# humansensinglab/AGenDA

Hardware: AMD Instinct MI355X
Metric: 512x512 images/sec + DAAM heatmaps, 50 DDIM steps, SD-1.5 (higher is better)
Workload: dtype bf16

## Files before the change

### agenda_amd/_lib.py

```python
from __future__ import annotations

import ctypes as C
import os

_HERE = os.path.dirname(os.path.abspath(__file__))
LIB_PATH = os.environ.get("AGD_LIB") or os.path.join(_HERE, "libagenda_hip.so")
AGD_MAX_LEVELS = 8
AGD_N_CLASSES = 11


class AgdConfig(C.Structure):
    _fields_ = [
        ("struct_size", C.c_int),
        ("in_channels", C.c_int), ("out_channels", C.c_int), ("n_levels", C.c_int),
        ("block_out_channels", C.c_int * AGD_MAX_LEVELS),
        ("down_cross", C.c_int * AGD_MAX_LEVELS),
        ("num_heads", C.c_int * AGD_MAX_LEVELS),
        ("layers_per_block", C.c_int), ("cross_attention_dim", C.c_int),
        ("use_linear_projection", C.c_int), ("norm_num_groups", C.c_int),
        ("vae_latent_channels", C.c_int), ("vae_out_channels", C.c_int), ("vae_n_levels", C.c_int),
        ("vae_block_out_channels", C.c_int * AGD_MAX_LEVELS),
        ("vae_layers_per_block", C.c_int), ("vae_norm_num_groups", C.c_int),
        ("vae_scaling_factor", C.c_float),
        ("max_tokens", C.c_int),
# ... 158 lines not shown
    "agd_hook_num_maps": (C.c_int, [_P]),
    "agd_hook_map_dims": (C.c_int, [_P, C.c_int, C.POINTER(C.c_int)]),
    "agd_hook_map": (C.c_int, [_P, C.c_int, _P, _P]),
    "agd_op_attn_reg_loss": (C.c_int, [_P, C.c_int, C.c_int, C.c_int, _P, _P, _P, C.c_float, _P, _P, _P]),
    "agd_attn_processor_backward": (C.c_int, [_P, C.c_char_p, _P, _P, _P, _P, C.c_int, C.c_int, C.c_int, C.c_int, _P, _P, _P]),
    "agd_op_conv2d": (C.c_int, [_P, _P, _P, _P] + [C.c_int] * 9 + [_P]),
    "agd_op_conv2d_ex": (C.c_int, [_P, _P, _P, _P] + [C.c_int] * 10 + [_P]),
    "agd_op_linear": (C.c_int, [_P, _P, _P, _P, _P, C.c_int, C.c_int, C.c_int, C.c_int, _P]),
    "agd_op_groupnorm": (C.c_int, [_P, _P, _P, _P, C.c_int, C.c_int, C.c_int, C.c_int, C.c_float, C.c_int, _P]),
    "agd_op_groupnorm_ex": (C.c_int, [_P] * 5 + [C.c_int] * 5 + [C.c_float, C.c_int, _P, C.c_int, _P, C.c_int, C.POINTER(C.c_int), _P]),
    "agd_op_gn_fold": (C.c_int, [_P, _P] + [C.c_int] * 5 + [C.c_float] + [_P] * 4 + [C.c_int, C.c_int] + [_P] * 5 + [_P]),
    "agd_op_conv_groupnorm": (C.c_int, [_P] * 6 + [C.c_int] * 6 + [C.c_float, C.c_int, C.c_int, _P]),
    "agd_op_igemm": (C.c_int, [C.POINTER(AgdIgemmDesc), _P]),
    "agd_op_layernorm": (C.c_int, [_P, _P, _P, _P, C.c_int, C.c_int, C.c_float, _P]),
    "agd_op_layernorm_ex": (C.c_int, [_P, _P, _P, _P, C.c_int, C.c_int, C.c_float, C.POINTER(C.c_int), _P]),
    "agd_op_ff_fused": (C.c_int, [_P] * 8 + [C.c_int, C.c_int, C.c_float, _P]),
    "agd_op_attn_chain": (C.c_int, [_P] * 9 + [C.c_int] * 5 + [C.c_float, _P]),
    "agd_op_ff_fused_ex": (C.c_int, [_P] * 8 + [C.c_int, C.c_int, C.c_float, _P, _P, _P, C.c_int, _P, C.c_int, _P, C.c_int, _P]),
    "agd_op_attn_chain_ex": (C.c_int, [_P] * 8 + [C.c_int] * 5 + [C.c_float] + [_P] * 4 + [C.c_int, _P, _P] + [C.c_int] * 6 + [_P]),
    "agd_op_qkv_chain": (C.c_int, [_P] * 3 + [C.c_int, C.c_float, _P, C.c_int] + [_P] * 4 + [C.c_float] + [_P] * 3 + [C.c_int] * 4 + [_P]),
    "agd_op_xattn_premul": (C.c_int, [_P] * 9 + [C.c_int] * 5 + [C.c_float, _P]),
    "agd_op_attention": (C.c_int, [_P, _P, _P, _P, C.c_int, C.c_int, C.c_int, C.c_int, C.c_int, C.c_float, _P, _P]),
    "agd_op_attention_ex": (C.c_int, [_P, _P, _P, _P] + [C.c_int] * 5 + [C.c_float, C.c_int, _P, _P, _P, C.c_int, C.c_int, _P, C.c_int, C.c_int, C.c_int, _P]),
    "agd_op_attention_long": (C.c_int, [_P, _P, _P, _P] + [C.c_int] * 5 + [C.c_float, C.c_int, _P, C.c_int, C.c_int, _P]),
    "agd_op_attention_headsum": (C.c_int, [_P, _P, _P, _P, C.c_int, C.c_int, C.c_int, C.c_int, C.c_int, C.c_float, _P, _P]),
    "agd_op_attention_backward": (C.c_int, [_P, _P, _P, _P] + [C.c_int] * 6 + [C.c_float, _P, _P, _P]),
    "agd_op_hook_headmean": (C.c_int, [_P, C.c_int, C.c_int, C.c_int, C.c_int, _P, _P]),
    "agd_op_bicubic_clamp_mean": (C.c_int, [_P, C.c_int, C.c_int, C.c_int, C.c_int, _P, _P]),
    "agd_op_heatmap_u8": (C.c_int, [_P, C.c_int, C.c_int, _P, _P]),
    "agd_op_resize_u8_pil": (C.c_int, [_P, C.c_int, C.c_int, C.c_int, C.c_int, C.c_int, C.c_int, _P, _P]),
    "agd_op_stack_heatmaps": (C.c_int, [_P, _P, _P, C.c_longlong, _P, _P, _P]),
    "agd_op_window_gather": (C.c_int, [_P, _P] + [C.c_int] * 8 + [_P]),
    "agd_op_window_mean": (C.c_int, [_P, _P] + [C.c_int] * 6 + [_P]),
    "agd_denoise_panorama": (C.c_int, [_P, _P] + [C.c_int] * 7 + [C.POINTER(C.c_float)] * 3 + [C.c_float, _P]),
    "agd_daam_global_panorama": (C.c_int, [_P, C.c_int, C.c_int, _P, _P]),
    "agd_op_region_masks": (C.c_int, [_P, C.c_int, C.c_int, _P] + [C.c_int] * 6 + [_P]),
    "agd_op_region_spread": (C.c_int, [_P] * 5 + [C.c_int] * 6 + [C.POINTER(C.c_int), C.c_float, C.c_float, _P]),
    "agd_op_region_mean": (C.c_int, [_P, _P, _P] + [C.c_int] * 5 + [_P]),
    "agd_denoise_regions": (C.c_int, [_P, _P, C.c_int, C.c_int, C.c_int, C.POINTER(AgdRegionsDesc), C.c_int] + [C.POINTER(C.c_float)] * 3 + [C.c_float, _P]),
    "agd_freeu_set": (C.c_int, [_P] + [C.c_float] * 4),
    "agd_freeu_clear": (C.c_int, [_P]),
    "agd_freeu_counts": (C.c_int, [_P, C.POINTER(C.c_longlong)]),
    "agd_op_freeu": (C.c_int, [_P, _P, _P, _P] + [C.c_int] * 5 + [C.c_float, C.c_float, _P]),
    "agd_guidance_rescale_set": (C.c_int, [_P, C.c_float]),
    "agd_guidance_rescale_clear": (C.c_int, [_P]),
    "agd_guidance_rescale_counts": (C.c_int, [_P, C.POINTER(C.c_longlong)]),
# ... 56 lines not shown
```

### agenda_amd/csrc/attention.hip

```cpp
#include "kernels.h"
#include <type_traits>

#ifdef AGD_EXPERIMENTS
int g_attn_qb = 1;
extern "C" __attribute__((visibility("default"))) void agd_set_attn_qb(int v) { g_attn_qb = v; }
#else
constexpr int g_attn_qb = 1;
#endif

template <int D> struct AttnCfg {
  static constexpr int KSTEPS = (D + 15) / 16;
  static constexpr int DBLK = (D + 31) / 32;
  static constexpr int KCH = KSTEPS * 2;
  static constexpr int KPITCH = ((KCH | 1)) * 16;
  static constexpr int VPITCH = ((DBLK | 1)) * 64;
  static constexpr int CH = D / 8;
  static constexpr bool ONES = (DBLK * 32 > D);
  static constexpr bool QPAD = (KSTEPS * 16 > D);
};

#define DEFER_THR 8.0f

template <int D, int KB, int QB, int RECORD, int AMASK = 0, int EXTRA = 0>
#if defined(AGD_EXPERIMENTS) && defined(EXP_ATTN_LB)
#define ATTN_LB(def) ((!RECORD && !AMASK) ? EXP_ATTN_LB : (def))
#else
#define ATTN_LB(def) (def)
#endif
__global__ __launch_bounds__(256, ATTN_LB((AMASK ? 1 : (QB == 1 && D <= 64 && !RECORD) ? 3 : (QB == 1 && D <= 80) ? 2 : 1))) void attn_kernel(const AttnP p) {
  using C = AttnCfg<D>;
  constexpr int KEYS = KB * 32;
  constexpr int KSTEPS = C::KSTEPS, DBLK = C::DBLK, KPITCH = C::KPITCH, VPITCH = C::VPITCH, CH = C::CH;
  constexpr bool ONES = C::ONES && !RECORD;
  constexpr bool QPAD = C::QPAD && !RECORD;
  constexpr bool CNEG = !QPAD && !RECORD;
  constexpr int NCHUNK = KEYS * CH;
  constexpr int LD_IT = (NCHUNK + 255) / 256;
  constexpr int STAGE = KEYS * (KPITCH + VPITCH);
  constexpr int NSTAGE = (RECORD == 1) ? 1 : 2;
  extern __shared__ __attribute__((aligned(16))) char smem[];

  const int tid = threadIdx.x, lane = tid & 63, wid = tid >> 6;
  const int c = lane & 31, hh = lane >> 5;
  const int HPB = (RECORD == 2) ? p.H / p.rec_hpb : p.H;
  const int nqt = p.nqt, nbh = p.B * HPB;
  int bh, qt;
  {
    const int id = blockIdx.x, x = id & 7, j = id >> 3;
    const int per = (nbh + 7) >> 3;
    const int lb = j / nqt;
    qt = j - lb * nqt;
    bh = x * per + lb;
  }
  if (bh >= nbh) return;
  const int hgrp = bh % HPB;
  int head = (RECORD == 2) ? hgrp * p.rec_hpb : hgrp;
  const int hend = (RECORD == 2) ? head + p.rec_hpb : head + 1;
  const int b = bh / HPB;
  const int q0 = qt * (128 * QB) + wid * (32 * QB);
  const bf16_t* kp = p.k + b * p.sk + head * D;
  const bf16_t* vp = p.v + b * p.sv + head * D;

// ... 41 lines not shown
    const bf16_t* qp = p.q + b * p.sq + h * D;
    const int qrow = q0 + c;
#pragma unroll
    for (int s = 0; s < (RECORD == 2 ? KSTEPS : 1); ++s) {
      const int d0 = 16 * s + 8 * hh;
      qnext[s] = u32x4{0, 0, 0, 0};
      if (qrow < p.Nq && d0 < D) qnext[s] = *(const u32x4*)(qp + (long long)qrow * p.ldq + d0);
    }
  };
  load_q();

  u32x4 kreg[LD_IT], vreg[LD_IT];
  unsigned kvoff[LD_IT], vvoff[LD_IT];
#pragma unroll
  for (int it = 0; it < LD_IT; ++it) {
    const int idx = tid + it * 256;
    const int r = idx / CH, cc = idx - r * CH;
    kvoff[it] = (idx < NCHUNK) ? (unsigned)((r * p.ldk + cc * 8) * 2) : 0x80000000u;
    vvoff[it] = (idx < NCHUNK) ? (unsigned)((r * p.ldv + cc * 8) * 2) : 0x80000000u;
  }
  const unsigned k_bytes = (unsigned)(((long long)(p.Nk - 1) * p.ldk + D) * 2), v_bytes = (unsigned)(((long long)(p.Nk - 1) * p.ldv + D) * 2);
  const auto krs = __builtin_amdgcn_make_buffer_rsrc((void*)kp, 0, k_bytes, 0x00020000);
  const auto vrs = __builtin_amdgcn_make_buffer_rsrc((void*)vp, 0, v_bytes, 0x00020000);
  auto gload = [&](int tile) {
    const unsigned ks_ = __builtin_amdgcn_readfirstlane((unsigned)(tile * KEYS * p.ldk * 2));
    const unsigned vs_ = __builtin_amdgcn_readfirstlane((unsigned)(tile * KEYS * p.ldv * 2));
#pragma unroll
    for (int it = 0; it < LD_IT; ++it) {
      kreg[it] = __builtin_bit_cast(u32x4, __builtin_amdgcn_raw_buffer_load_b128(krs, kvoff[it], ks_, 0));
      vreg[it] = __builtin_bit_cast(u32x4, __builtin_amdgcn_raw_buffer_load_b128(vrs, vvoff[it], vs_, 0));
    }
  };
  auto gload_head = [&](int h) {
    const auto krh = __builtin_amdgcn_make_buffer_rsrc((void*)(p.k + b * p.sk + h * D), 0, k_bytes, 0x00020000);
    const auto vrh = __builtin_amdgcn_make_buffer_rsrc((void*)(p.v + b * p.sv + h * D), 0, v_bytes, 0x00020000);
#pragma unroll
    for (int it = 0; it < LD_IT; ++it) {
      kreg[it] = __builtin_bit_cast(u32x4, __builtin_amdgcn_raw_buffer_load_b128(krh, kvoff[it], 0, 0));
      vreg[it] = __builtin_bit_cast(u32x4, __builtin_amdgcn_raw_buffer_load_b128(vrh, vvoff[it], 0, 0));
    }
  };
  auto gload_extra = [&]() {
    const unsigned k2b = (unsigned)(((long long)(p.Nk2 - 1) * p.ldk2 + D) * 2), v2b = (unsigned)(((long long)(p.Nk2 - 1) * p.ldv2 + D) * 2);
    const auto kr2 = __builtin_amdgcn_make_buffer_rsrc((void*)(p.k2 + b * p.sk2 + head * D), 0, k2b, 0x00020000);
    const auto vr2 = __builtin_amdgcn_make_buffer_rsrc((void*)(p.v2 + b * p.sv2 + head * D), 0, v2b, 0x00020000);
#pragma unroll
// ... 30 lines not shown
  float m_run[QB], l_run[QB];
  [[maybe_unused]] bool seen[QB];
  f32x16 negm[CNEG ? QB : 1];
#pragma unroll
  for (int qb = 0; qb < QB; ++qb) {
    m_run[qb] = RECORD ? -INFINITY : 0.f; l_run[qb] = 0.f; seen[qb] = false;
    if constexpr (CNEG) {
#pragma unroll
      for (int j = 0; j < 16; ++j) negm[qb][j] = 0.f;
    }
  }
  const float sc = qscale;
  f32x16 pacc[RECORD == 2 ? KB : 1];
  const bool recb = RECORD == 2 && p.record_mode == 3 && b >= p.rec_b0;
  if constexpr (RECORD == 2) {
#pragma unroll
    for (int kb = 0; kb < KB; ++kb)
#pragma unroll
      for (int j = 0; j < 16; ++j) pacc[kb][j] = 0.f;
  }

  const int ntiles_main = RECORD ? 1 : (p.Nk + KEYS - 1) / KEYS;
  const int ntiles = ntiles_main + (EXTRA ? 1 : 0);
  const bool ragged = (p.Nk % KEYS) != 0 || p.causal || AMASK;
  gload(0);
  lstore(0);
  __syncthreads();

  const int gi = lane & 15;
  const int tr_row = (gi >> 2) + 4 * hh;
  const int tr_col = ((lane >> 4) & 1) * 16 + (gi & 3) * 4;

  auto tile_body = [&](int t, auto mask_tag) {
    constexpr bool MASK = decltype(mask_tag)::value;
    const int cur = (RECORD == 1) ? 0 : (RECORD == 2) ? ((t - (hend - p.rec_hpb)) & 1) : (t & 1);
    const char* sK = smem + cur * STAGE;
    const char* sV = sK + KEYS * KPITCH;
    if constexpr (RECORD == 2) { if (t + 1 < hend) { gload_head(t + 1); prefetch_q(t + 1); } }
    else if constexpr (EXTRA) { if (t + 1 < ntiles_main) gload(t + 1); else if (t + 1 == ntiles_main) gload_extra(); }
    else if (t + 1 < ntiles) gload(t + 1);
    f32x16 sacc[QB][KB];
#pragma unroll
    for (int kb = 0; kb < KB; ++kb) {
#pragma unroll
      for (int s = 0; s < KSTEPS; ++s) {
        const bf16x8 a = *(const bf16x8*)(sK + (kb * 32 + c) * KPITCH + (2 * s + hh) * 16);
#pragma unroll
        for (int qb = 0; qb < QB; ++qb) {
          if (s == 0) { const f32x16 z = {0.f, 0.f, 0.f, 0.f, 0.f, 0.f, 0.f, 0.f, 0.f, 0.f, 0.f, 0.f, 0.f, 0.f, 0.f, 0.f};
                        sacc[qb][kb] = __builtin_amdgcn_mfma_f32_32x32x16_bf16(a, qf[qb][s], CNEG ? negm[qb] : z, 0, 0, 0); }
          else sacc[qb][kb] = __builtin_amdgcn_mfma_f32_32x32x16_bf16(a, qf[qb][s], sacc[qb][kb], 0, 0, 0);
        }
      }
    }
    if constexpr (MASK) {
#pragma unroll
      for (int qb = 0; qb < QB; ++qb)
#pragma unroll
        for (int kb = 0; kb < KB; ++kb)
#pragma unroll
          for (int i = 0; i < 16; ++i) {
            const int key = (RECORD || (EXTRA && t == ntiles_main) ? 0 : t * KEYS) + kb * 32 + (i & 3) + 8 * (i >> 2) + 4 * hh;
// ... 95 lines not shown
          float* base = p.rec + img * p.rec_img_stride + head * p.rec_head_stride;
          const unsigned nbytes = (unsigned)p.rec_T * (unsigned)p.Nq * 4u;
          const auto rsrc = __builtin_amdgcn_make_buffer_rsrc(base, 0, nbytes, 0x00020000);
          const unsigned rowb = (unsigned)p.Nq * 4u;
          const unsigned voff0 = (unsigned)(q0 + c) * 4u + (unsigned)(4 * hh) * rowb;
#pragma unroll
          for (int kb = 0; kb < KB; ++kb) {
            float old[16];
#pragma unroll
            for (int i = 0; i < 16; ++i) {
              const unsigned off = voff0 + (unsigned)(kb * 32 + (i & 3) + 8 * (i >> 2)) * rowb;
              old[i] = __builtin_bit_cast(float, __builtin_amdgcn_raw_buffer_load_b32(rsrc, off, 0, 0));
            }
#pragma unroll
            for (int i = 0; i < 16; ++i) {
              const unsigned off = voff0 + (unsigned)(kb * 32 + (i & 3) + 8 * (i >> 2)) * rowb;
              __builtin_amdgcn_raw_buffer_store_b32(__builtin_bit_cast(unsigned, old[i] + sacc[0][kb][i] * inv), rsrc, off, 0, 0);
            }
          }
        }
      }
    }

#pragma unroll
    for (int kb = 0; kb < KB; ++kb)
#pragma unroll
      for (int s = 0; s < 2; ++s) {
        bf16x8 pf[QB];
#pragma unroll
        for (int qb = 0; qb < QB; ++qb)
#pragma unroll
          for (int j = 0; j < 8; ++j) pf[qb][j] = (__bf16)sacc[qb][kb][8 * s + j];
        const char* vb = sV + (kb * 32 + 16 * s + tr_row) * VPITCH + tr_col * 2;
#pragma unroll
        for (int db = 0; db < DBLK; ++db) {
          const s16x4 lo = __builtin_amdgcn_ds_read_tr16_b64_v4i16((__attribute__((address_space(3))) s16x4*)(vb + db * 64));
          const s16x4 hi = __builtin_amdgcn_ds_read_tr16_b64_v4i16((__attribute__((address_space(3))) s16x4*)(vb + 8 * VPITCH + db * 64));
          const u32x2 lo2 = __builtin_bit_cast(u32x2, lo), hi2 = __builtin_bit_cast(u32x2, hi);
          const u32x4 a4 = u32x4{lo2[0], lo2[1], hi2[0], hi2[1]};
#pragma unroll
          for (int qb = 0; qb < QB; ++qb)
            oacc[qb][db] = __builtin_amdgcn_mfma_f32_32x32x16_bf16(__builtin_bit_cast(bf16x8, a4), pf[qb], oacc[qb][db], 0, 0, 0);
        }
      }
    if ((RECORD == 2) ? (t + 1 < hend) : (t + 1 < ntiles)) {
      lstore(cur ^ 1);
      __syncthreads();
    }
  };
  auto store_o = [&]() {
#pragma unroll
    for (int qb = 0; qb < QB; ++qb) {
      float lt;
      if constexpr (ONES) {
        constexpr int ld = D % 32;
        const float lv = oacc[qb][D / 32][4 * (ld / 8)];
        lt = __shfl(lv, c);
      } else {
        lt = xhalf_sum(l_run[qb]);
      }
      const float inv = 1.0f / lt;
      const int qrow = q0 + qb * 32 + c;
      if (qrow < p.Nq) {
        bf16_t* op = p.o + b * p.so + (long long)qrow * p.ldo + head * D;
#pragma unroll
        for (int db = 0; db < DBLK; ++db)
#pragma unroll
          for (int g = 0; g < 4; ++g) {
            const int d0 = db * 32 + 8 * g + 4 * hh;
// ... 39 lines not shown
        for (int kb = 0; kb < KB; ++kb)
#pragma unroll
          for (int i = 0; i < 16; ++i)
            __builtin_amdgcn_raw_buffer_store_b32(__builtin_bit_cast(unsigned, old[kb][i] + pacc[kb][i]), rsrc,
                                                  voff0 + (unsigned)(kb * 32 + (i & 3) + 8 * (i >> 2)) * rowb, 0, 0);
      }
      return;
    } else if constexpr (RECORD) {
      tile_body(0, T_{});
    } else if constexpr (EXTRA) {
      for (int t = 0; t < ntiles_main - 1; ++t) tile_body(t, F_{});
      if (ragged) tile_body(ntiles_main - 1, T_{}); else tile_body(ntiles_main - 1, F_{});
      tile_body(ntiles_main, T_{});
    } else {
      if (p.causal || AMASK) { for (int t = 0; t < ntiles - 1; ++t) tile_body(t, T_{}); }
      else { for (int t = 0; t < ntiles - 1; ++t) tile_body(t, F_{}); }
      if (ragged) tile_body(ntiles - 1, T_{}); else tile_body(ntiles - 1, F_{});
    }
  }
  store_o();
}


template <int D, int KB, int QB, int RECORD, int AMASK = 0, int EXTRA = 0>
static int launch_attn_t(const AttnP& p, hipStream_t st) {
  using C = AttnCfg<D>;
  constexpr int lds = (RECORD == 1 ? 1 : 2) * KB * 32 * (C::KPITCH + C::VPITCH);
  AttnP pp = p;
  pp.nqt = (p.Nq + 128 * QB - 1) / (128 * QB);
  const int per = (p.B * (RECORD == 2 ? p.H / p.rec_hpb : p.H) + 7) / 8;
  dim3 grid(8 * per * pp.nqt);
  auto kfn = attn_kernel<D, KB, QB, RECORD, AMASK, EXTRA>;
  if (lds > 65536) {
    static std::atomic<bool> attr[AGD_MAX_DEVICES] = {};
    int dev = 0; HIP_CHECK_RET(hipGetDevice(&dev));
    if (dev < 0 || dev >= AGD_MAX_DEVICES) { agd_set_error("attention: device ordinal %d out of range", dev); return -1; }
    if (!attr[dev]) { HIP_CHECK_RET(hipFuncSetAttribute((const void*)kfn, hipFuncAttributeMaxDynamicSharedMemorySize, lds)); attr[dev] = true; }
  }
  hipLaunchKernelGGL(kfn, grid, dim3(256), lds, st, pp);
  HIP_CHECK_RET(hipGetLastError());
  return 0;
}

template <int D>
static int launch_attn_d(const AttnP& p, hipStream_t st) {
  if (p.k2) {
    if (p.record_mode != 0 || p.mask || p.causal) { agd_set_error("attention: a second K/V source takes no recording, mask or causal order"); return -1; }
    if (!p.v2 || p.Nk2 < 1 || p.Nk2 > 64 || ((p.ldk2 | p.ldv2) & 7)) { agd_set_error("attention: second K/V source of %d keys (1 .. 64, pitches multiples of 8)", p.Nk2); return -1; }
    return launch_attn_t<D, 2, 1, 0, 0, 1>(p, st);
  }
  if (p.record_mode != 0) {
    if (p.Nk > 96) { agd_set_error("attention: recording needs Nk <= 96 (got %d)", p.Nk); return -1; }
    if (p.record_mode == 3) {
      if (p.mask) { agd_set_error("attention: head-summed recording does not take an attention mask"); return -1; }
      if (p.rec_hpb < 1 || p.H % p.rec_hpb) { agd_set_error("attention: rec_hpb %d does not divide %d heads", p.rec_hpb, p.H); return -1; }
      return launch_attn_t<D, 3, 1, 2>(p, st);
    }
    return p.mask ? launch_attn_t<D, 3, 1, 1, 1>(p, st) : launch_attn_t<D, 3, 1, 1>(p, st);
  }
  if (p.mask) {
    if (p.causal) { agd_set_error("attention: additive mask + causal unsupported"); return -1; }
    return (p.Nk <= 96 && p.Nk > 64) ? launch_attn_t<D, 3, 1, 0, 1>(p, st) : launch_attn_t<D, 2, 1, 0, 1>(p, st);
  }
  if (p.Nk <= 96 && p.Nk > 64) return launch_attn_t<D, 3, 1, 0>(p, st);
  if constexpr (D <= 80) { if (p.Nq >= 1024 && g_attn_qb == 2) return launch_attn_t<D, 2, 2, 0>(p, st); }
#if defined(AGD_EXPERIMENTS) && defined(EXP_ATTN_KB)
  if (p.Nk >= 1024) return launch_attn_t<D, EXP_ATTN_KB, 1, 0>(p, st);
#endif
  return launch_attn_t<D, 2, 1, 0>(p, st);
}

int launch_attention(const AttnP& p, hipStream_t st) {
  if ((p.ldq | p.ldk | p.ldv | p.ldo) & 3) { agd_set_error("attention: row pitches must be multiples of 4 elements"); return -1; }
  if ((p.ldq | p.ldk | p.ldv) & 7) { agd_set_error("attention: q/k/v pitches must be multiples of 8 elements"); return -1; }
  switch (p.D) {
    case 32: return launch_attn_d<32>(p, st);
    case 40: return launch_attn_d<40>(p, st);
    case 64: return launch_attn_d<64>(p, st);
    case 80: return launch_attn_d<80>(p, st);
    case 128: return launch_attn_d<128>(p, st);
    case 160: return launch_attn_d<160>(p, st);
    default: agd_set_error("attention: unsupported head dim %d", p.D); return -1;
  }
}
```

### agenda_amd/csrc/kernels.h

```cpp
#pragma once
#include "common.h"

#define AGD_MAX_DEVICES 16
struct SplitKWs { float* p = nullptr; size_t cap = 0; };

struct IgemmP {
  const bf16_t* sc0 = nullptr; const bf16_t* sc1 = nullptr; int sc_C0 = 0, sc_C1 = 0;
  int ups4 = 0;
  const bf16_t* src0; const bf16_t* src1;
  int C0, C1;
  int Hin, Win, Hout, Wout;
  int ksize, stride, pad, up;
  const bf16_t* W;
  const float* bias; int bias_mode;
  const float* rowadd; int rowadd_ld;
  const bf16_t* residual; int ldr;
  void* out; int out_f32; int ldo;
  int M, N, K;
  float alpha;
  int geglu;
  int act;
  int batch;
  long long sA0, sA1, sW, sO, sR;
  const bf16_t* zero_page;
// ... 22 lines not shown
  int* ran;
};
enum { IGEMM_RAN_NONE = 0, IGEMM_RAN_GENERAL = 1, IGEMM_RAN_HALO = 2, IGEMM_RAN_PCH = 3, IGEMM_RAN_PC = 4, IGEMM_RAN_8P = 5, IGEMM_RAN_SMAP = 6, IGEMM_RAN_WREG = 7 };
enum { IGEMM_SLAB_NONE = 0, IGEMM_SLAB_PLAIN = 1, IGEMM_SLAB_GN = 2 };
int launch_igemm(const IgemmP& p, hipStream_t st);
int igemm_query(const IgemmP& p, int* cfg3);

struct AttnP {
  const bf16_t* q; const bf16_t* k; const bf16_t* v; bf16_t* o;
  int ldq, ldk, ldv, ldo;
  long long sq, sk, sv, so;
  int B, H, D, Nq, Nk;
  float scale;
  int record_mode; int rec_b0;
  float* rec; long long rec_img_stride; long long rec_head_stride;
  int rec_T;
  int rec_hpb;
  int nqt;
  int causal;
  const float* mask;
  const bf16_t* k2; const bf16_t* v2; int ldk2, ldv2; long long sk2, sv2; int Nk2;
};
int launch_attention(const AttnP& p, hipStream_t st);
constexpr int ATTN_LONG_MAX_KEYS = 320;
int launch_attention_long(const AttnP& p, hipStream_t st);

struct FFusedP {
  const bf16_t* h; bf16_t* out;
  const bf16_t* w1f;
  const float* cs1; const float* b1;
  const bf16_t* w2f;
  const float* b2;
  int M; float ln_eps;
  const bf16_t* wpf; const float* bp; const bf16_t* xres; bf16_t* pout; float* colstat;
  int xres_rows;
  int premul;
};
int launch_ff_fused(const FFusedP& p, int C, hipStream_t st);
struct AttnChainP {
  const bf16_t* h; bf16_t* out;
  const float* gamma; const float* beta; float ln_eps;
  const bf16_t* wqf;
  const bf16_t* wof; const float* bo;
  const bf16_t* kv; int ldkv; long long skv;
  int M, HW, T; float scale;
  int record; float* rec; long long rec_img_stride, rec_head_stride; int rec_T, rec_b0, rec_hpb;
// ... 179 lines not shown
```

### agenda_amd/csrc/model.hip

```cpp
#include "../../include/agenda_hip.h"
#include "kernels.h"

#include <algorithm>
#include <cmath>
#include <cstdarg>
#include <cstdio>
#include <cstring>
#include <functional>
#include <string>
#include <unordered_map>
#include <unordered_set>
#include <vector>

static thread_local char g_err[2048] = "";
#define AGD_API extern "C" __attribute__((visibility("default")))
extern "C" void agd_set_error(const char* fmt, ...) {
  va_list ap; va_start(ap, fmt); vsnprintf(g_err, sizeof(g_err), fmt, ap); va_end(ap);
}
#define CK(expr) do { if ((expr) != 0) return -1; } while (0)
#define FAIL(...) do { agd_set_error(__VA_ARGS__); return -1; } while (0)

struct WMat { bf16_t* w = nullptr; int N = 0, Cin = 0, Cpad = 0, taps = 0;
              int sc_cols = 0;
              bf16_t* wfrag = nullptr; int wfrag_ni = 0; };
// ... 2580 lines not shown
}

AGD_API int agd_set_option(agd_ctx* c, const char* name, int value) {
  if (!c || !name) { agd_set_error("set_option: null argument"); return fail_ctx(c); }
  if (!strcmp(name, "cfg_shared_prefix")) { c->opt_cfg_share = value != 0; return 0; }
  if (!strcmp(name, "ln_fold")) { c->opt_ln_fold = value; return 0; }
  if (!strcmp(name, "gn_fused_stats")) { c->opt_gn_fused = value != 0; return 0; }
  if (!strcmp(name, "weight_touch")) { c->opt_touch = value < 0 ? 0 : value; return 0; }
  if (!strcmp(name, "weight_warm")) { c->opt_warm = value; return 0; }
  if (!strcmp(name, "conv_halo")) { c->opt_halo = value != 0; return 0; }
  if (!strcmp(name, "gn_proj_fold")) { c->opt_gn_proj_fold = value < 0 ? 0 : value; return 0; }
  if (!strcmp(name, "tblock_fuse")) { c->opt_tb_fuse = value < 0 ? 0 : value; return 0; }
  if (!strcmp(name, "reduce_gn")) { c->opt_reduce_gn = value != 0; return 0; }
  if (!strcmp(name, "xcd_block")) { c->opt_xcd_block = value != 0; return 0; }
  if (!strcmp(name, "igemm_pc")) { c->opt_pc = value < 0 ? 0 : value; return 0; }
  if (!strcmp(name, "attn2_premul")) { c->opt_xpre = value < 0 ? 0 : value; return 0; }
  if (!strcmp(name, "conv_smap")) { c->opt_smap = value != 0; return 0; }
  if (!strcmp(name, "side_stream")) { c->opt_side = value < 0 ? 0 : value; return 0; }
  if (!strcmp(name, "igemm_kgroups")) { c->opt_kg2 = value != 0; return 0; }
  if (!strcmp(name, "upsample_phases")) { c->opt_ups4 = value & 15; return 0; }
  if (!strcmp(name, "ff_proj_fuse")) { c->opt_ffproj = value != 0; return 0; }
  if (!strcmp(name, "shortcut_fuse")) { c->opt_sc_fuse = value & 3; return 0; }
  if (!strcmp(name, "wreg_mask")) { c->opt_wreg = value & 3; return 0; }
  if (!strcmp(name, "igemm8p")) { c->opt_p8 = value < 0 ? 0 : value; return 0; }
  agd_set_error("set_option: unknown option '%s'", name);
  return fail_ctx(c);
}

AGD_API int agd_record_config(agd_ctx* c, int mode, int is_train, int rec_tokens) {
  if (!c) return -1;
  if (mode < 0 || mode > 2) { agd_set_error("record_config: mode %d", mode); return fail_ctx(c); }
  c->rec_mode = mode; c->rec_is_train = is_train; c->rec_T_cfg = rec_tokens;
  return 0;
}

static int hook_reset_rows(agd_ctx* c, int rows, int L, hipStream_t st) {
  const int Tc = c->ctx_T > 0 ? c->ctx_T : c->cfg.max_tokens;
  const size_t n = (size_t)rows * Tc * L * L;
  CK(c->hook_sumb.ensure(n * 4)); CK(c->hook_scratchb.ensure(n * 4));
  c->hook_sum = c->hook_sumb.as<float>(); c->hook_scratch = c->hook_scratchb.as<float>();
  c->hook_Bp = rows; c->hook_T = Tc;
  if (hipMemsetAsync(c->hook_sum, 0, n * 4, st) != hipSuccess) FAIL("memset hook");
  c->hook_count = 0; c->hook_recs.clear(); c->hook_store_used = 0;
  return 0;
}

// ... 683 lines not shown
  CK(launch_f32_to_bf16(kv, kvb, (long long)B * T * 2 * C, st));
  CK(launch_convert_weight(wq, wqb, C, C, 1, C, 0, st)); CK(launch_transpose_bf16(wqb, C, C, wqT, st));
  CK(launch_convert_weight(wo, wob, C, C, 1, C, 0, st));
  CK(launch_matvec_bf16(wqb, beta, wqbeta, C, C, st));
  CK(launch_rowstat_bf16(xb, rst, (int)M, C, st));
  XattnPremulP pm{}; pm.kv = kvb; pm.ldkv = 2 * C; pm.skv = (long long)T * 2 * C; pm.wqT = wqT; pm.wo = wob; pm.gamma = gamma; pm.wqb = wqbeta;
  pm.B = B; pm.T = T; pm.C = C; pm.H = heads; pm.scale = 1.0f / sqrtf((float)(C / heads)); pm.kpp = kpp; pm.kcs = kcs; pm.kbs = kcs + (size_t)B * HT; pm.vpp = vpp;
  CK(launch_xattn_premul(pm, st));
  XattnSP sp{}; sp.x = xb; sp.ln_stats = rst; sp.ln_slots = 1; sp.ln_invC = 1.0f / (float)C; sp.ln_eps = eps; sp.kpp = kpp; sp.kcs = pm.kcs; sp.kbs = pm.kbs; sp.P = P;
  sp.M = (int)M; sp.HW = HW; sp.C = C; sp.H = heads; sp.T = T;
  if (probs) {
    if (hipMemsetAsync(probs, 0, (size_t)B * heads * T * HW * 4, st) != hipSuccess) { agd_set_error("memset probs"); return -1; }
    sp.rec = probs; sp.rec_b0 = 0; sp.rec_T = T; sp.rec_head_stride = (long long)T * HW; sp.rec_img_stride = sp.rec_head_stride * heads;
  }
  CK(launch_xattn_s(sp, st));
  WMat wv; wv.w = vpp; wv.N = C; wv.Cin = (int)HT; wv.Cpad = (int)HT; wv.taps = 1;
  GemmOpt oo; oo.bias = bo; oo.residual = xb; oo.w_per_image = 1;
  CK(run_conv(nullptr, st, P, (int)HT, nullptr, 0, B, 1, HW, wv, 1, yb, oo, op_zero_page()));
  CK(launch_bf16_to_f32(yb, y, M * C, st));
  hipStreamSynchronize(st);
  return 0;
}

AGD_API int agd_op_attention(const float* q, const float* k, const float* v, float* o, int B, int H, int D, int Nq, int Nk,
                                float scale, float* probs_out, void* stream) {
  hipStream_t st = S(stream); Tmp tmp;
  const int C = H * D;
  bf16_t* qb = tmp.get<bf16_t>((size_t)B * Nq * C); bf16_t* kb = tmp.get<bf16_t>((size_t)B * Nk * C);
  bf16_t* vb = tmp.get<bf16_t>((size_t)B * Nk * C); bf16_t* ob = tmp.get<bf16_t>((size_t)B * Nq * C);
  if (!qb || !kb || !vb || !ob) return -1;
  CK(launch_f32_to_bf16(q, qb, (long long)B * Nq * C, st));
  CK(launch_f32_to_bf16(k, kb, (long long)B * Nk * C, st));
  CK(launch_f32_to_bf16(v, vb, (long long)B * Nk * C, st));
  AttnP a{}; a.q = qb; a.k = kb; a.v = vb; a.o = ob; a.ldq = a.ldk = a.ldv = a.ldo = C;
  a.sq = (long long)Nq * C; a.so = a.sq; a.sk = (long long)Nk * C; a.sv = a.sk;
  a.B = B; a.H = H; a.D = D; a.Nq = Nq; a.Nk = Nk; a.scale = scale;
  if (probs_out) {
    if (hipMemsetAsync(probs_out, 0, (size_t)B * H * Nk * Nq * 4, st) != hipSuccess) { agd_set_error("memset probs"); return -1; }
    a.record_mode = 1; a.rec_b0 = 0; a.rec = probs_out; a.rec_T = Nk;
    a.rec_head_stride = (long long)Nk * Nq; a.rec_img_stride = a.rec_head_stride * H;
  }
  CK(launch_attention(a, st));
  CK(launch_bf16_to_f32(ob, o, (long long)B * Nq * C, st));
  hipStreamSynchronize(st);
  return 0;
}

AGD_API int agd_op_attention_ex(const float* q, const float* k, const float* v, float* o, int B, int H, int D, int Nq, int Nk, float scale,
                                int causal, const float* mask, const float* k2, const float* v2, int Nk2, int layout, float* probs_out,
                                int record, int rec_b0, int rec_T, void* stream) {
  if (D != 32 && D != 40 && D != 64 && D != 80 && D != 128 && D != 160) { agd_set_error("attention_ex: unsupported head dim D=%d", D); return -1; }
  if (B < 1 || H < 1 || Nq < 1 || Nk < 1) { agd_set_error("attention_ex: bad shape B=%d H=%d Nq=%d Nk=%d", B, H, Nq, Nk); return -1; }
  if (!q || !k || !v || !o) { agd_set_error("attention_ex: q, k, v and o are required"); return -1; }
  if (layout < 0 || layout > 2) { agd_set_error("attention_ex: layout=%d (0 packed, 1 fused q|k|v rows, 2 fused k|v rows)", layout); return -1; }
  if (layout == 1 && Nq != Nk) { agd_set_error("attention_ex: layout=1 (fused q|k|v rows) needs Nq == Nk (got Nq=%d Nk=%d)", Nq, Nk); return -1; }
  if (record < 0 || record > 2 || (record != 0) != (probs_out != nullptr)) { agd_set_error("attention_ex: record=%d needs probs_out, and probs_out needs record 1 or 2", record); return -1; }
  if (record && Nk > 96) { agd_set_error("attention_ex: recording needs Nk <= 96 (got Nk=%d)", Nk); return -1; }
  if (record && (rec_b0 < 0 || rec_b0 > B)) { agd_set_error("attention_ex: rec_b0=%d outside [0, %d]", rec_b0, B); return -1; }
  if (record && (rec_T < 1 || rec_T > Nk)) { agd_set_error("attention_ex: rec_T=%d outside [1, %d]", rec_T, Nk); return -1; }
  if ((k2 != nullptr) != (v2 != nullptr)) { agd_set_error("attention_ex: k2 and v2 come together"); return -1; }
  if (!k2 && Nk2 != 0) { agd_set_error("attention_ex: Nk2=%d without a second source", Nk2); return -1; }
  hipStream_t st = S(stream); Tmp tmp;
  const int C = H * D;
  const long long nq = (long long)B * Nq * C, nk = (long long)B * Nk * C, nk2 = k2 ? (long long)B * (Nk2 > 0 ? Nk2 : 0) * C : 0;
  bf16_t* qb = tmp.get<bf16_t>((size_t)nq); bf16_t* kb = tmp.get<bf16_t>((size_t)nk); bf16_t* vb = tmp.get<bf16_t>((size_t)nk);
  bf16_t* ob = tmp.get<bf16_t>((size_t)nq);
  bf16_t* k2b = k2 ? tmp.get<bf16_t>((size_t)nk2 + 8) : nullptr; bf16_t* v2b = k2 ? tmp.get<bf16_t>((size_t)nk2 + 8) : nullptr;
  bf16_t* fused = layout ? tmp.get<bf16_t>((size_t)(layout == 1 ? 3 : 2) * nk) : nullptr;
  bf16_t* fused2 = (layout && k2) ? tmp.get<bf16_t>((size_t)2 * nk2 + 8) : nullptr;
  if (!qb || !kb || !vb || !ob || (k2 && (!k2b || !v2b)) || (layout && !fused) || (layout && k2 && !fused2)) return -1;
  CK(launch_f32_to_bf16(q, qb, nq, st));
  CK(launch_f32_to_bf16(k, kb, nk, st));
  CK(launch_f32_to_bf16(v, vb, nk, st));
  if (nk2 > 0) { CK(launch_f32_to_bf16(k2, k2b, nk2, st)); CK(launch_f32_to_bf16(v2, v2b, nk2, st)); }
  auto place = [&](bf16_t* dst, int wide, int col, const bf16_t* src, long long rows) {
    if (rows < 1) return 0;
    if (hipMemcpy2DAsync(dst + (size_t)col * C, (size_t)wide * C * 2, src, (size_t)C * 2, (size_t)C * 2, (size_t)rows, hipMemcpyDeviceToDevice, st) != hipSuccess) {
      agd_set_error("attention_ex: layout copy failed"); return -1; }
    return 0;
  };
  AttnP a{}; a.q = qb; a.k = kb; a.v = vb; a.o = ob; a.ldq = a.ldk = a.ldv = a.ldo = C;
  a.sq = (long long)Nq * C; a.so = a.sq; a.sk = (long long)Nk * C; a.sv = a.sk;
  if (layout == 1) {
    CK(place(fused, 3, 0, qb, (long long)B * Nq)); CK(place(fused, 3, 1, kb, (long long)B * Nk)); CK(place(fused, 3, 2, vb, (long long)B * Nk));
    a.q = fused; a.k = fused + C; a.v = fused + 2 * C; a.ldq = a.ldk = a.ldv = 3 * C; a.sq = a.sk = a.sv = (long long)Nk * 3 * C;
  } else if (layout == 2) {
    CK(place(fused, 2, 0, kb, (long long)B * Nk)); CK(place(fused, 2, 1, vb, (long long)B * Nk));
    a.k = fused; a.v = fused + C; a.ldk = a.ldv = 2 * C; a.sk = a.sv = (long long)Nk * 2 * C;
  }
  a.B = B; a.H = H; a.D = D; a.Nq = Nq; a.Nk = Nk; a.scale = scale; a.causal = causal ? 1 : 0; a.mask = mask;
  if (k2) {
    a.k2 = k2b; a.v2 = v2b; a.ldk2 = a.ldv2 = C; a.sk2 = a.sv2 = (long long)Nk2 * C; a.Nk2 = Nk2;
    if (layout) {
// ... 1578 lines not shown
```

### agenda_amd/ops.py

```python
from __future__ import annotations

import ctypes

import torch

from . import _lib


def _f32c(t):
    assert t.is_cuda, "ops run on the GPU only (no CPU fallback)"
    return t.detach().to(torch.float32).contiguous()


_P8 = {0: 0, 1: 2, 2: 4, 3: 8}


def conv2d(x, w, bias=None, stride=1, padding=None, upsample=False, halo=False, p8=0, smap=False, phases=False, pc=0, xcd_block=False):
    lib = _lib.load()
    x, w = _f32c(x), _f32c(w)
    b = _f32c(bias) if bias is not None else None
    B, Cin, H, W = x.shape
    Cout, _, k, _ = w.shape
    pad = (1 if k == 3 else 0) if padding is None else padding
    up = 2 if upsample else 1
# ... 320 lines not shown
            raise ValueError(f"attention: k {tuple(k.shape)} / v {tuple(v.shape)} must both be [B, Nk, H*D] = [{B}, Nk, {Cc}]")
        if mask is not None and tuple(mask.shape) != (B, Nk):
            raise ValueError(f"attention: mask {tuple(mask.shape)} must be {(B, Nk)}")
        if (k2 is None) != (v2 is None) or (k2 is not None and (k2.shape != v2.shape or k2.ndim != 3 or k2.shape[0] != B or k2.shape[2] != Cc)):
            raise ValueError("attention: k2 and v2 come together, both [B, Nk2, H*D]")
        if head_sum and not return_probs:
            raise ValueError("attention: head_sum is a form of return_probs")
        Nk2 = 0 if k2 is None else k2.shape[1]
        probs = None
        if return_probs:
            probs = torch.empty((B, max(Nk, 1), max(Nq, 1)) if head_sum else (B, heads, max(Nk, 1), max(Nq, 1)), device=q.device, dtype=torch.float32)
        _lib.check(lib.agd_op_attention_ex(_lib.ptr(_given(q)), _lib.ptr(_given(k)), _lib.ptr(_given(v)), _lib.ptr(_given(o)), B, heads, D, Nq, Nk, float(scale),
                                           int(bool(causal)), _lib.ptr(None if mask is None else _given(mask)),
                                           _lib.ptr(None if k2 is None else _given(k2)), _lib.ptr(None if v2 is None else _given(v2)), Nk2, int(layout),
                                           _lib.ptr(probs), (2 if head_sum else 1) if return_probs else 0, int(rec_b0),
                                           Nk if rec_T is None else int(rec_T), _lib.current_stream_ptr()), None, "agd_op_attention_ex")
        return (o, probs) if return_probs else o
    probs = torch.empty(B, heads, Nk, Nq, device=q.device, dtype=torch.float32) if return_probs else None
    _lib.check(lib.agd_op_attention(_lib.ptr(q), _lib.ptr(k), _lib.ptr(v), _lib.ptr(o), B, heads, D, Nq, Nk, float(scale),
                                    _lib.ptr(probs), _lib.current_stream_ptr()), None, "agd_op_attention")
    return (o, probs) if return_probs else o


def attention_long(q, k, v, heads, scale=None, *, layout=0, rec_b0=0, rec_T=None, probs=None):
    lib = _lib.load()
    q, k, v = _f32c(q), _f32c(k), _f32c(v)
    B, Nq, Cc = q.shape
    Nk = k.shape[1]
    if k.shape != (B, Nk, Cc) or v.shape != k.shape:
        raise ValueError(f"attention_long: k {tuple(k.shape)} / v {tuple(v.shape)} must both be [B, Nk, H*D] = [{B}, Nk, {Cc}]")
    D = Cc // heads
    scale = D ** -0.5 if scale is None else scale
    o = torch.empty_like(q)
    if probs is None:
        probs = torch.zeros(B, heads, max(Nk, 1), max(Nq, 1), device=q.device, dtype=torch.float32)
    elif tuple(probs.shape) != (B, heads, Nk, Nq) or probs.dtype != torch.float32 or not probs.is_contiguous() or not probs.is_cuda:
        raise ValueError(f"attention_long: probs must be a contiguous fp32 GPU tensor {(B, heads, Nk, Nq)}")
    _lib.check(lib.agd_op_attention_long(_lib.ptr(_given(q)), _lib.ptr(_given(k)), _lib.ptr(_given(v)), _lib.ptr(_given(o)), B, heads, D, Nq, Nk,
                                         float(scale), int(layout), _lib.ptr(probs), int(rec_b0), Nk if rec_T is None else int(rec_T),
                                         _lib.current_stream_ptr()), None, "agd_op_attention_long")
    return o, probs


def attention_headsum(q, k, v, heads, scale=None):
    lib = _lib.load()
    q, k, v = _f32c(q), _f32c(k), _f32c(v)
# ... 238 lines not shown
```

### include/agenda_hip.h

```cpp
#ifndef AGENDA_HIP_H
#define AGENDA_HIP_H
#ifdef __cplusplus
extern "C" {
#endif

typedef struct agd_ctx agd_ctx;

#define AGD_MAX_LEVELS 8

typedef struct agd_config {
  int struct_size;
  int in_channels, out_channels, n_levels;
  int block_out_channels[AGD_MAX_LEVELS];
  int down_cross[AGD_MAX_LEVELS];
  int num_heads[AGD_MAX_LEVELS];
  int layers_per_block, cross_attention_dim, use_linear_projection, norm_num_groups;
  int vae_latent_channels, vae_out_channels, vae_n_levels;
  int vae_block_out_channels[AGD_MAX_LEVELS];
  int vae_layers_per_block, vae_norm_num_groups;
  float vae_scaling_factor;
  int max_tokens;
  int prediction_type;
  long long workspace_bytes;
  int text_hidden, text_layers, text_heads, text_intermediate, text_vocab, text_max_pos;
// ... 206 lines not shown
  int batch;
  int rowstat_slots, ln_slots, colstat_rows;
  int gn_groups, gn_silu, gn_keep_out;
  int halo, p8, smap, pc, kg2, wreg, xcd_block;
  float alpha, ln_invC, ln_eps, gn_eps;
  long long sA0, sA1, sW, sO, sR;
  long long n_src0, n_src1, n_sc0, n_sc1, n_w, n_res, n_out;
  const float* src0; const float* src1; const float* sc0; const float* sc1; const float* w;
  const float* bias; const float* rowadd; const float* residual;
  const float* ln_stats; const float* ln_cs; const float* gn_gamma; const float* gn_beta;
  float* out; float* gn_y; float* rowstat; float* colstat;
  int cfg[3]; int ran[2]; int gn_fused; int can_fuse_sc;
} agd_igemm_desc;
int agd_op_igemm(agd_igemm_desc* d, void* stream);
int agd_op_layernorm(const float* x, const float* gamma, const float* beta, float* y, int rows, int C, float eps,
                     void* stream);
int agd_op_layernorm_ex(const float* x, const float* gamma, const float* beta, float* y, int rows, int C, float eps, int* inst,
                        void* stream);
int agd_op_attention(const float* q, const float* k, const float* v, float* o, int B, int H, int D, int Nq, int Nk,
                     float scale, float* probs_out, void* stream);
int agd_op_attention_ex(const float* q, const float* k, const float* v, float* o, int B, int H, int D, int Nq, int Nk, float scale,
                        int causal, const float* mask, const float* k2, const float* v2, int Nk2, int layout, float* probs_out,
                        int record, int rec_b0, int rec_T, void* stream);
int agd_op_attention_long(const float* q, const float* k, const float* v, float* o, int B, int H, int D, int Nq, int Nk, float scale,
                          int layout, float* probs_inout, int rec_b0, int rec_T, void* stream);
int agd_op_attention_headsum(const float* q, const float* k, const float* v, float* o, int B, int H, int D, int Nq, int Nk,
                             float scale, float* probs_sum_out, void* stream);
int agd_op_attention_backward(const float* q, const float* kv, const float* d_o, const float* d_map, int b0, int B, int H, int D,
                              int N, int T, float scale, float* dq, float* dkv, void* stream);
int agd_op_hook_headmean(const float* heads, int Bp, int H, int T, int N, float* map, void* stream);
int agd_op_bicubic_clamp_mean(const float* maps, int n_maps, int T, int side, int S, float* out, void* stream);

int agd_op_heatmap_u8(const float* hm, int n, int npix, unsigned char* out, void* stream);
int agd_op_resize_u8_pil(const unsigned char* in, int n, int H, int W, int C, int oh, int ow, unsigned char* out, void* stream);
int agd_op_stack_heatmaps(const unsigned char* obj, const unsigned char* fg, const unsigned char* bg, long long npix,
                          unsigned char* rgb, unsigned char* inv, void* stream);

int agd_lora_add(agd_ctx* ctx, const char* target_key, const float* down, const float* up, int rank, float alpha);
int agd_lora_set_scale(agd_ctx* ctx, float s, void* stream);
int agd_lora_clear(agd_ctx* ctx);
int agd_lora_count(agd_ctx* ctx);
float agd_lora_scale(agd_ctx* ctx);

int agd_op_window_gather(const float* canvas, float* views, int B, int C, int Lh, int Lw, int window, int stride, int v0, int n, void* stream);
int agd_op_window_mean(const float* views, float* canvas, int B, int C, int Lh, int Lw, int window, int stride, void* stream);
int agd_denoise_panorama(agd_ctx* ctx, float* canvas, int batch, int Lh, int Lw, int window, int stride, int view_batch, int n_steps,
// ... 68 lines not shown
```

Baseline: 8.926.

## Stage flash-attention K/V via LDS-DMA buffer loads and transposed LDS reads

Adds a DMA variant of the 64-key flash attention kernel for head dims 40 and 80. It loads K/V tiles straight from global memory into LDS with buffer DMA instead of going through registers, and reads V with ds_read_b64_tr_b16 transposed loads for the PV MFMA. It also raises occupancy bounds for these variants. The goal is to cut register staging and LDS store traffic and to overlap the next tile's load with compute. The cost is that every tile is treated as ragged (masked), and K/V scratch buffers get NaN-filled tail padding with extra memsets.

```diff
diff --git a/agenda_amd/_lib.py b/agenda_amd/_lib.py
--- a/agenda_amd/_lib.py
+++ b/agenda_amd/_lib.py
@@ -204,6 +204,7 @@
     "agd_op_xattn_premul": (C.c_int, [_P] * 9 + [C.c_int] * 5 + [C.c_float, _P]),
     "agd_op_attention": (C.c_int, [_P, _P, _P, _P, C.c_int, C.c_int, C.c_int, C.c_int, C.c_int, C.c_float, _P, _P]),
     "agd_op_attention_ex": (C.c_int, [_P, _P, _P, _P] + [C.c_int] * 5 + [C.c_float, C.c_int, _P, _P, _P, C.c_int, C.c_int, _P, C.c_int, C.c_int, C.c_int, _P]),
+    "agd_op_attention_dma": (C.c_int, [C.c_int]),
     "agd_op_attention_long": (C.c_int, [_P, _P, _P, _P] + [C.c_int] * 5 + [C.c_float, C.c_int, _P, C.c_int, C.c_int, _P]),
     "agd_op_attention_headsum": (C.c_int, [_P, _P, _P, _P, C.c_int, C.c_int, C.c_int, C.c_int, C.c_int, C.c_float, _P, _P]),
     "agd_op_attention_backward": (C.c_int, [_P, _P, _P, _P] + [C.c_int] * 6 + [C.c_float, _P, _P, _P]),
diff --git a/agenda_amd/csrc/attention.hip b/agenda_amd/csrc/attention.hip
--- a/agenda_amd/csrc/attention.hip
+++ b/agenda_amd/csrc/attention.hip
@@ -19,15 +19,30 @@
   static constexpr bool QPAD = (KSTEPS * 16 > D);
 };
 
+#define ATTN_DMA_WON 3
+static std::atomic<int> g_attn_dma{ATTN_DMA_WON};
+void attention_set_dma(int v) { g_attn_dma = v <= 0 ? 0 : v == 1 ? ATTN_DMA_WON : 3; }
+
+template <int OFF> AGD_DEV u32x2 tr_read(unsigned addr) {
+  u32x2 r;
+  asm volatile("ds_read_b64_tr_b16 %0, %1 offset:%2" : "=v"(r) : "v"(addr), "i"(OFF) : "memory");
+  return r;
+}
+template <int N, int DB> AGD_DEV void tr_wait(u32x2 (&lo)[DB], u32x2 (&hi)[DB]) {
+  static_assert(DB == 2 || DB == 3, "PV d-blocks of the LDS-DMA kernels");
+  if constexpr (DB == 2) asm volatile("s_waitcnt lgkmcnt(%4)" : "+v"(lo[0]), "+v"(hi[0]), "+v"(lo[1]), "+v"(hi[1]) : "i"(N));
+  else asm volatile("s_waitcnt lgkmcnt(%6)" : "+v"(lo[0]), "+v"(hi[0]), "+v"(lo[1]), "+v"(hi[1]), "+v"(lo[2]), "+v"(hi[2]) : "i"(N));
+}
+
 #define DEFER_THR 8.0f
 
-template <int D, int KB, int QB, int RECORD, int AMASK = 0, int EXTRA = 0>
+template <int D, int KB, int QB, int RECORD, int AMASK = 0, int EXTRA = 0, int DMA = 0>
 #if defined(AGD_EXPERIMENTS) && defined(EXP_ATTN_LB)
 #define ATTN_LB(def) ((!RECORD && !AMASK) ? EXP_ATTN_LB : (def))
 #else
 #define ATTN_LB(def) (def)
 #endif
-__global__ __launch_bounds__(256, ATTN_LB((AMASK ? 1 : (QB == 1 && D <= 64 && !RECORD) ? 3 : (QB == 1 && D <= 80) ? 2 : 1))) void attn_kernel(const AttnP p) {
+__global__ __launch_bounds__(256, ATTN_LB((AMASK ? 1 : (DMA && D <= 64) ? 4 : (DMA && D <= 80) ? 3 : (QB == 1 && D <= 64 && !RECORD) ? 3 : (QB == 1 && D <= 80) ? 2 : 1))) void attn_kernel(const AttnP p) {
   using C = AttnCfg<D>;
   constexpr int KEYS = KB * 32;
   constexpr int KSTEPS = C::KSTEPS, DBLK = C::DBLK, KPITCH = C::KPITCH, VPITCH = C::VPITCH, CH = C::CH;
@@ -38,6 +53,8 @@
   constexpr int LD_IT = (NCHUNK + 255) / 256;
   constexpr int STAGE = KEYS * (KPITCH + VPITCH);
   constexpr int NSTAGE = (RECORD == 1) ? 1 : 2;
+  constexpr int KP = KPITCH / 16, VP = VPITCH / 16, K_IT = (KP + 3) / 4, V_IT = VP / 4;
+  static_assert(!DMA || (KB == 2 && QB == 1 && !RECORD && !AMASK && !EXTRA && VP % 4 == 0), "LDS-DMA staging: the plain 64-key flash kernel only");
   extern __shared__ __attribute__((aligned(16))) char smem[];
 
   const int tid = threadIdx.x, lane = tid & 63, wid = tid >> 6;
@@ -125,6 +142,34 @@
   const unsigned k_bytes = (unsigned)(((long long)(p.Nk - 1) * p.ldk + D) * 2), v_bytes = (unsigned)(((long long)(p.Nk - 1) * p.ldv + D) * 2);
   const auto krs = __builtin_amdgcn_make_buffer_rsrc((void*)kp, 0, k_bytes, 0x00020000);
   const auto vrs = __builtin_amdgcn_make_buffer_rsrc((void*)vp, 0, v_bytes, 0x00020000);
+  const int wu = __builtin_amdgcn_readfirstlane(wid);
+  unsigned kdoff[DMA ? K_IT : 1], vdoff[DMA ? V_IT : 1];
+  if constexpr (DMA) {
+#pragma unroll
+    for (int i = 0; i < K_IT; ++i) {
+      const int g = (wid + 4 * i) * 64 + lane, r = g / KP, cc = g - r * KP;
+      kdoff[i] = (cc < CH) ? (unsigned)((r * p.ldk + cc * 8) * 2) : 0x80000000u;
+    }
+#pragma unroll
+    for (int i = 0; i < V_IT; ++i) {
+      const int g = i * 64 + lane, r = g / VP, cc = g - r * VP;
+      vdoff[i] = (cc < CH) ? (unsigned)(((16 * wid + r) * p.ldv + cc * 8) * 2) : 0x80000000u;
+    }
+  }
+  auto gload_dma = [&](int tile, int stage) {
+    char* dK = smem + stage * STAGE;
+    char* dV = dK + KEYS * KPITCH;
+    const long long ko = (long long)tile * KEYS * p.ldk, vo = (long long)tile * KEYS * p.ldv;
+    const bf16_t* kt = kp + ko;
+    const bf16_t* vt = vp + vo;
+    const unsigned kn = k_bytes - (unsigned)(ko * 2), vn = v_bytes - (unsigned)(vo * 2);
+#pragma unroll
+    for (int i = 0; i < (DMA ? K_IT : 0); ++i)
+      if ((i + 1) * 4 <= KP || wu + 4 * i < KP) { if (kdoff[i] != 0x80000000u) bufdma16(kt, dK + (wu + 4 * i) * 1024, kdoff[i], 0u, kn); }
+#pragma unroll
+    for (int i = 0; i < (DMA ? V_IT : 0); ++i) { if (vdoff[i] != 0x80000000u) bufdma16(vt, dV + (wu * V_IT + i) * 1024, vdoff[i], 0u, vn); }
+  };
+  auto dma_landed = [&]() { asm volatile("s_waitcnt vmcnt(0)" ::: "memory"); };
   auto gload = [&](int tile) {
     const unsigned ks_ = __builtin_amdgcn_readfirstlane((unsigned)(tile * KEYS * p.ldk * 2));
     const unsigned vs_ = __builtin_amdgcn_readfirstlane((unsigned)(tile * KEYS * p.ldv * 2));
@@ -201,9 +246,9 @@
 
   const int ntiles_main = RECORD ? 1 : (p.Nk + KEYS - 1) / KEYS;
   const int ntiles = ntiles_main + (EXTRA ? 1 : 0);
-  const bool ragged = (p.Nk % KEYS) != 0 || p.causal || AMASK;
-  gload(0);
-  lstore(0);
+  const bool ragged = DMA || (p.Nk % KEYS) != 0 || p.causal || AMASK;
+  if constexpr (DMA) { gload_dma(0, 0); dma_landed(); }
+  else { gload(0); lstore(0); }
   __syncthreads();
 
   const int gi = lane & 15;
@@ -215,8 +260,12 @@
     const int cur = (RECORD == 1) ? 0 : (RECORD == 2) ? ((t - (hend - p.rec_hpb)) & 1) : (t & 1);
     const char* sK = smem + cur * STAGE;
     const char* sV = sK + KEYS * KPITCH;
+    if constexpr (DMA) {
+      if constexpr (MASK) asm volatile("; masked tile" ::: "memory"); else asm volatile("; plain tile" ::: "memory");
+    }
     if constexpr (RECORD == 2) { if (t + 1 < hend) { gload_head(t + 1); prefetch_q(t + 1); } }
     else if constexpr (EXTRA) { if (t + 1 < ntiles_main) gload(t + 1); else if (t + 1 == ntiles_main) gload_extra(); }
+    else if constexpr (DMA) { if (t + 1 < ntiles) gload_dma(t + 1, cur ^ 1); }
     else if (t + 1 < ntiles) gload(t + 1);
     f32x16 sacc[QB][KB];
 #pragma unroll
@@ -358,6 +407,35 @@
       }
     }
 
+    if constexpr (DMA) {
+      constexpr int NG = KB * 2;
+      const unsigned va = (unsigned)(unsigned long long)((__attribute__((address_space(3))) const char*)sV) + (unsigned)(tr_row * VPITCH + tr_col * 2);
+      u32x2 lo[2][DBLK], hi[2][DBLK];
+      auto issue = [&](auto g_tag) {
+        constexpr int g = decltype(g_tag)::value, base = (g >> 1) * 32 * VPITCH + (g & 1) * 16 * VPITCH;
+        static_assert(base + 8 * VPITCH + (DBLK - 1) * 64 < 65536, "ds offset field");
+        if constexpr (DBLK >= 1) { lo[g & 1][0] = tr_read<base>(va); hi[g & 1][0] = tr_read<base + 8 * VPITCH>(va); }
+        if constexpr (DBLK >= 2) { lo[g & 1][1] = tr_read<base + 64>(va); hi[g & 1][1] = tr_read<base + 8 * VPITCH + 64>(va); }
+        if constexpr (DBLK >= 3) { lo[g & 1][2] = tr_read<base + 128>(va); hi[g & 1][2] = tr_read<base + 8 * VPITCH + 128>(va); }
+      };
+      auto group = [&](auto g_tag) {
+        constexpr int g = decltype(g_tag)::value, kb = g >> 1, s = g & 1;
+        if constexpr (g + 1 < NG) { issue(std::integral_constant<int, g + 1>{}); tr_wait<2 * DBLK>(lo[g & 1], hi[g & 1]); }
+        else tr_wait<0>(lo[g & 1], hi[g & 1]);
+        bf16x8 pf;
+#pragma unroll
+        for (int j = 0; j < 8; ++j) pf[j] = (__bf16)sacc[0][kb][8 * s + j];
+#pragma unroll
+        for (int db = 0; db < DBLK; ++db) {
+          const u32x4 a4 = u32x4{lo[g & 1][db][0], lo[g & 1][db][1], hi[g & 1][db][0], hi[g & 1][db][1]};
+          oacc[0][db] = __builtin_amdgcn_mfma_f32_32x32x16_bf16(__builtin_bit_cast(bf16x8, a4), pf, oacc[0][db], 0, 0, 0);
+        }
+      };
+      issue(std::integral_constant<int, 0>{});
+      group(std::integral_constant<int, 0>{}); group(std::integral_constant<int, 1>{});
+      group(std::integral_constant<int, 2>{}); group(std::integral_constant<int, 3>{});
+      static_assert(NG == 4, "LDS-DMA kernels: KB = 2");
+    } else
 #pragma unroll
     for (int kb = 0; kb < KB; ++kb)
 #pragma unroll
@@ -380,7 +458,8 @@
         }
       }
     if ((RECORD == 2) ? (t + 1 < hend) : (t + 1 < ntiles)) {
-      lstore(cur ^ 1);
+      if constexpr (DMA) dma_landed();
+      else lstore(cur ^ 1);
       __syncthreads();
     }
   };
@@ -466,7 +545,7 @@
 }
 
 
-template <int D, int KB, int QB, int RECORD, int AMASK = 0, int EXTRA = 0>
+template <int D, int KB, int QB, int RECORD, int AMASK = 0, int EXTRA = 0, int DMA = 0>
 static int launch_attn_t(const AttnP& p, hipStream_t st) {
   using C = AttnCfg<D>;
   constexpr int lds = (RECORD == 1 ? 1 : 2) * KB * 32 * (C::KPITCH + C::VPITCH);
@@ -474,7 +553,7 @@
   pp.nqt = (p.Nq + 128 * QB - 1) / (128 * QB);
   const int per = (p.B * (RECORD == 2 ? p.H / p.rec_hpb : p.H) + 7) / 8;
   dim3 grid(8 * per * pp.nqt);
-  auto kfn = attn_kernel<D, KB, QB, RECORD, AMASK, EXTRA>;
+  auto kfn = attn_kernel<D, KB, QB, RECORD, AMASK, EXTRA, DMA>;
   if (lds > 65536) {
     static std::atomic<bool> attr[AGD_MAX_DEVICES] = {};
     int dev = 0; HIP_CHECK_RET(hipGetDevice(&dev));
@@ -511,6 +590,7 @@
 #if defined(AGD_EXPERIMENTS) && defined(EXP_ATTN_KB)
   if (p.Nk >= 1024) return launch_attn_t<D, EXP_ATTN_KB, 1, 0>(p, st);
 #endif
+  if constexpr (D == 40 || D == 80) { if (g_attn_dma & (D == 40 ? 1 : 2)) return launch_attn_t<D, 2, 1, 0, 0, 0, 1>(p, st); }
   return launch_attn_t<D, 2, 1, 0>(p, st);
 }
 
diff --git a/agenda_amd/csrc/kernels.h b/agenda_amd/csrc/kernels.h
--- a/agenda_amd/csrc/kernels.h
+++ b/agenda_amd/csrc/kernels.h
@@ -68,6 +68,7 @@
   const bf16_t* k2; const bf16_t* v2; int ldk2, ldv2; long long sk2, sv2; int Nk2;
 };
 int launch_attention(const AttnP& p, hipStream_t st);
+void attention_set_dma(int v);
 constexpr int ATTN_LONG_MAX_KEYS = 320;
 int launch_attention_long(const AttnP& p, hipStream_t st);
 
diff --git a/agenda_amd/csrc/model.hip b/agenda_amd/csrc/model.hip
--- a/agenda_amd/csrc/model.hip
+++ b/agenda_amd/csrc/model.hip
@@ -2626,6 +2626,7 @@
   if (!strcmp(name, "ff_proj_fuse")) { c->opt_ffproj = value != 0; return 0; }
   if (!strcmp(name, "shortcut_fuse")) { c->opt_sc_fuse = value & 3; return 0; }
   if (!strcmp(name, "wreg_mask")) { c->opt_wreg = value & 3; return 0; }
+  if (!strcmp(name, "attn_dma")) { attention_set_dma(value); return 0; }
   if (!strcmp(name, "igemm8p")) { c->opt_p8 = value < 0 ? 0 : value; return 0; }
   agd_set_error("set_option: unknown option '%s'", name);
   return fail_ctx(c);
@@ -3355,13 +3356,23 @@
   return 0;
 }
 
+AGD_API int agd_op_attention_dma(int value) { attention_set_dma(value); return 0; }
+
+constexpr int ATTN_TAIL_ROWS = 64;
+static int attn_nan_tail(bf16_t* end, size_t elems, hipStream_t st) {
+  if (hipMemsetAsync(end, 0xFF, elems * 2, st) != hipSuccess) { agd_set_error("attention: tail memset failed"); return -1; }
+  return 0;
+}
+
 AGD_API int agd_op_attention(const float* q, const float* k, const float* v, float* o, int B, int H, int D, int Nq, int Nk,
                                 float scale, float* probs_out, void* stream) {
   hipStream_t st = S(stream); Tmp tmp;
   const int C = H * D;
-  bf16_t* qb = tmp.get<bf16_t>((size_t)B * Nq * C); bf16_t* kb = tmp.get<bf16_t>((size_t)B * Nk * C);
-  bf16_t* vb = tmp.get<bf16_t>((size_t)B * Nk * C); bf16_t* ob = tmp.get<bf16_t>((size_t)B * Nq * C);
+  const size_t tail = (size_t)ATTN_TAIL_ROWS * C;
+  bf16_t* qb = tmp.get<bf16_t>((size_t)B * Nq * C); bf16_t* kb = tmp.get<bf16_t>((size_t)B * Nk * C + tail);
+  bf16_t* vb = tmp.get<bf16_t>((size_t)B * Nk * C + tail); bf16_t* ob = tmp.get<bf16_t>((size_t)B * Nq * C);
   if (!qb || !kb || !vb || !ob) return -1;
+  CK(attn_nan_tail(kb + (size_t)B * Nk * C, tail, st)); CK(attn_nan_tail(vb + (size_t)B * Nk * C, tail, st));
   CK(launch_f32_to_bf16(q, qb, (long long)B * Nq * C, st));
   CK(launch_f32_to_bf16(k, kb, (long long)B * Nk * C, st));
   CK(launch_f32_to_bf16(v, vb, (long long)B * Nk * C, st));
@@ -3396,12 +3407,16 @@
   hipStream_t st = S(stream); Tmp tmp;
   const int C = H * D;
   const long long nq = (long long)B * Nq * C, nk = (long long)B * Nk * C, nk2 = k2 ? (long long)B * (Nk2 > 0 ? Nk2 : 0) * C : 0;
-  bf16_t* qb = tmp.get<bf16_t>((size_t)nq); bf16_t* kb = tmp.get<bf16_t>((size_t)nk); bf16_t* vb = tmp.get<bf16_t>((size_t)nk);
+  const size_t tail = (size_t)ATTN_TAIL_ROWS * C;
+  bf16_t* qb = tmp.get<bf16_t>((size_t)nq); bf16_t* kb = tmp.get<bf16_t>((size_t)nk + tail); bf16_t* vb = tmp.get<bf16_t>((size_t)nk + tail);
   bf16_t* ob = tmp.get<bf16_t>((size_t)nq);
   bf16_t* k2b = k2 ? tmp.get<bf16_t>((size_t)nk2 + 8) : nullptr; bf16_t* v2b = k2 ? tmp.get<bf16_t>((size_t)nk2 + 8) : nullptr;
-  bf16_t* fused = layout ? tmp.get<bf16_t>((size_t)(layout == 1 ? 3 : 2) * nk) : nullptr;
+  const size_t fwide = layout == 1 ? 3 : 2;
+  bf16_t* fused = layout ? tmp.get<bf16_t>(fwide * ((size_t)nk + tail)) : nullptr;
   bf16_t* fused2 = (layout && k2) ? tmp.get<bf16_t>((size_t)2 * nk2 + 8) : nullptr;
   if (!qb || !kb || !vb || !ob || (k2 && (!k2b || !v2b)) || (layout && !fused) || (layout && k2 && !fused2)) return -1;
+  CK(attn_nan_tail(kb + nk, tail, st)); CK(attn_nan_tail(vb + nk, tail, st));
+  if (layout) CK(attn_nan_tail(fused + fwide * (size_t)nk, fwide * tail, st));
   CK(launch_f32_to_bf16(q, qb, nq, st));
   CK(launch_f32_to_bf16(k, kb, nk, st));
   CK(launch_f32_to_bf16(v, vb, nk, st));
diff --git a/agenda_amd/ops.py b/agenda_amd/ops.py
--- a/agenda_amd/ops.py
+++ b/agenda_amd/ops.py
@@ -366,6 +366,10 @@
     return (o, probs) if return_probs else o
 
 
+def attention_dma(value):
+    _lib.check(_lib.load().agd_op_attention_dma(int(value)), None, "agd_op_attention_dma")
+
+
 def attention_long(q, k, v, heads, scale=None, *, layout=0, rec_b0=0, rec_T=None, probs=None):
     lib = _lib.load()
     q, k, v = _f32c(q), _f32c(k), _f32c(v)
diff --git a/include/agenda_hip.h b/include/agenda_hip.h
--- a/include/agenda_hip.h
+++ b/include/agenda_hip.h
@@ -252,6 +252,7 @@
 int agd_op_attention_ex(const float* q, const float* k, const float* v, float* o, int B, int H, int D, int Nq, int Nk, float scale,
                         int causal, const float* mask, const float* k2, const float* v2, int Nk2, int layout, float* probs_out,
                         int record, int rec_b0, int rec_T, void* stream);
+int agd_op_attention_dma(int value);
 int agd_op_attention_long(const float* q, const float* k, const float* v, float* o, int B, int H, int D, int Nq, int Nk, float scale,
                           int layout, float* probs_inout, int rec_b0, int rec_T, void* stream);
 int agd_op_attention_headsum(const float* q, const float* k, const float* v, float* o, int B, int H, int D, int Nq, int Nk,
```

After: 8.986, median of 6. About the same (+0.7%).
